# johnnyjana730/MVIN

Measured on AMD Instinct MI355X. Metric: (user,item) pairs scored/sec @ dim=64 hop=2 fan-out=32; % HBM roofline, higher is better.
Workload: dtype f32

## Files before the change

mvin_amd/csrc/mvin_fused_agg.hip:

```cpp
#include "mvin_fused_agg.h"

namespace mvin {

template <int K>
__global__ __launch_bounds__(kAggWaves * 64) void entity_aggregates_kernel(EntityAggArgs a) {
    constexpr int D = 64, SPL = K / 16;
    static_assert(K == 16 || K == 32 || K == 64, "K");
    extern __shared__ __attribute__((aligned(16))) float smem[];
    const int nRp = (a.nR + 3) & ~3;
    float* sT = smem;
    const int tid = threadIdx.x, lane = tid & 63, wave = tid >> 6;
    const int g = lane >> 4, c = lane & 15;
    unsigned* sLo = reinterpret_cast<unsigned*>(sT + nRp + wave * agg_list_words(K)) + g * (K + kAggPad);
    float* sLw = reinterpret_cast<float*>(reinterpret_cast<unsigned*>(sT + nRp + wave * agg_list_words(K)) + 4 * (K + kAggPad)) + g * (K + kAggPad);
    const bool att = a.t0 != nullptr;
    const float invK = 1.f / (float)K;
    const bool fast = agg_logit_table(a.t0, a.nR, sT, tid, lane);
    __syncthreads();

    const int tbytes = (int)a.table_bytes;
    const __amdgpu_buffer_rsrc_t tabS = __builtin_amdgcn_make_buffer_rsrc(const_cast<float*>(a.tabS), 0, tbytes, 0x00020000);
    const __amdgpu_buffer_rsrc_t tabG = __builtin_amdgcn_make_buffer_rsrc(const_cast<float*>(a.tabG), 0, tbytes, 0x00020000);
    const __amdgpu_buffer_rsrc_t selfS = __builtin_amdgcn_make_buffer_rsrc(const_cast<float*>(a.selfS), 0, a.selfS ? tbytes : 0, 0x00020000);
    const __amdgpu_buffer_rsrc_t selfG = __builtin_amdgcn_make_buffer_rsrc(const_cast<float*>(a.selfG), 0, tbytes, 0x00020000);
    const __amdgpu_buffer_rsrc_t adjE = __builtin_amdgcn_make_buffer_rsrc(const_cast<int32_t*>(a.adj_e), 0, (int)a.adj_bytes, 0x00020000);
    const __amdgpu_buffer_rsrc_t adjR = __builtin_amdgcn_make_buffer_rsrc(const_cast<int32_t*>(a.adj_r), 0, (int)a.adj_bytes, 0x00020000);
    const __amdgpu_buffer_rsrc_t outS = __builtin_amdgcn_make_buffer_rsrc(a.outS, 0, tbytes, 0x00020000);
    const __amdgpu_buffer_rsrc_t outG = __builtin_amdgcn_make_buffer_rsrc(a.outG, 0, tbytes, 0x00020000);
    const unsigned c16 = (unsigned)c * 16u;
    const unsigned n_entity = (unsigned)a.n_entity;
    const unsigned nquad = (n_entity + 3u) >> 2;

    auto run = [&](auto fast_tag) {
        constexpr bool FAST = decltype(fast_tag)::value;
        for (unsigned quad = blockIdx.x * kAggWaves + wave; quad < nquad; quad += gridDim.x * kAggWaves) {
            const unsigned e = quad * 4u + (unsigned)g;
            const bool valid = e < n_entity;
            unsigned ce[SPL], cr[SPL];
            agg_load_slots<SPL>(adjE, adjR, valid ? (e * (unsigned)K + (unsigned)(SPL * c)) * 4u : kAggOob, ce, cr);
            const unsigned so = valid ? e * (unsigned)(D * 4) + c16 : kAggPadRow;
            const float4 sg = agg_row4(selfG, so);
            const float4 ss = agg_row4(selfS, so);
            float wk[SPL];
            agg_row_weights<SPL, FAST>(cr, att, sT, (unsigned)(a.nR - 1), invK, wk);
            int cc = (int)(cr[0] >> 24);
            cc = valid ? (cc < 1 ? 1 : (cc > K ? K : cc)) : 0;
            __builtin_amdgcn_fence(__ATOMIC_RELEASE, "wavefront");
            __builtin_amdgcn_wave_barrier();
#pragma unroll
            for (int i = 0; i < SPL; ++i) {
                sLo[SPL * c + i] = ((cr[i] >> 16) & 0xFFu) ? (ce[i] & 0xFFFFFFu) * (unsigned)(D * 4) : kAggPadRow;
                sLw[SPL * c + i] = wk[i];
            }
            __builtin_amdgcn_fence(__ATOMIC_RELEASE, "wavefront");
            __builtin_amdgcn_wave_barrier();
            __builtin_amdgcn_fence(__ATOMIC_ACQUIRE, "wavefront");
            const int kmax = __builtin_amdgcn_readfirstlane(agg_xor32_imax(agg_xor16_imax(cc)));
            f32x2 s01 = {0.f, 0.f}, s23 = {0.f, 0.f}, g01 = {0.f, 0.f}, g23 = {0.f, 0.f};
            for (int k0 = 0; k0 < kmax; k0 += 4) {
                const uint4 o4 = *reinterpret_cast<const uint4*>(sLo + k0);
                const float4 w4 = *reinterpret_cast<const float4*>(sLw + k0);
                const unsigned off[4] = {o4.x, o4.y, o4.z, o4.w};
                const float ws_[4] = {w4.x, w4.y, w4.z, w4.w};
                float4 r1[4], r2[4];
#pragma unroll
                for (int t = 0; t < 4; ++t) {
                    r1[t] = agg_row4(tabS, off[t] + c16);
                    r2[t] = agg_row4(tabG, off[t] + c16);
                }
#pragma unroll
                for (int t = 0; t < 4; ++t) {
                    const f32x2 w2 = {ws_[t], ws_[t]};
                    s01 = __builtin_elementwise_fma(w2, f32x2{r1[t].x, r1[t].y}, s01);
                    s23 = __builtin_elementwise_fma(w2, f32x2{r1[t].z, r1[t].w}, s23);
                    g01 = __builtin_elementwise_fma(w2, f32x2{r2[t].x, r2[t].y}, g01);
                    g23 = __builtin_elementwise_fma(w2, f32x2{r2[t].z, r2[t].w}, g23);
                }
            }
            const unsigned oo = valid ? e * (unsigned)(D * 4) + c16 : kAggOob;
            const u32x4 vs = {__float_as_uint(s01[0] + ss.x), __float_as_uint(s01[1] + ss.y), __float_as_uint(s23[0] + ss.z),
                              __float_as_uint(s23[1] + ss.w)};
            const u32x4 vg = {__float_as_uint(g01[0] + sg.x), __float_as_uint(g01[1] + sg.y), __float_as_uint(g23[0] + sg.z),
                              __float_as_uint(g23[1] + sg.w)};
            __builtin_amdgcn_raw_buffer_store_b128(vs, outS, oo, 0, 0);
            __builtin_amdgcn_raw_buffer_store_b128(vg, outG, oo, 0, 0);
        }
    };
    if (fast) run(std::true_type{});
    else run(std::false_type{});
}

template <int K>
__global__ __launch_bounds__(kAggWaves * 64, K == 64 ? 3 : 4) void gather_attn_l2_agg_kernel(FusedL2Args a) {
    constexpr int D = 64, SPL = K / 16;
    static_assert(K == 16 || K == 32 || K == 64, "K");
    extern __shared__ __attribute__((aligned(16))) float smem[];
    const int nRp = (a.nR + 3) & ~3;
    float* sT = smem;
    const int tid = threadIdx.x, lane = tid & 63, wave = tid >> 6;
    const int g = lane >> 4, c = lane & 15;
    float* sUV = sT + nRp + wave * (16 * kAggUvLd + agg_list_words(K));
    unsigned* sLo = reinterpret_cast<unsigned*>(sUV + 16 * kAggUvLd) + g * (K + kAggPad);
    float* sLw = reinterpret_cast<float*>(reinterpret_cast<unsigned*>(sUV + 16 * kAggUvLd) + 4 * (K + kAggPad)) + g * (K + kAggPad);
    const bool att1 = a.t1 != nullptr;
    const float invK = 1.f / (float)K;
    const bool fold = a.fold != 0;
    const float c0 = fold ? 1.f : a.t0 != nullptr ? invK : 1.f;
    const bool fast = agg_logit_table(a.t1, a.nR, sT, tid, lane);
    __syncthreads();

    const unsigned tbytes = (unsigned)a.table_bytes;
    const __amdgpu_buffer_rsrc_t aggS = __builtin_amdgcn_make_buffer_rsrc(a.agg, 0, (int)tbytes, 0x00020000);
    const __amdgpu_buffer_rsrc_t aggG = __builtin_amdgcn_make_buffer_rsrc(reinterpret_cast<char*>(a.agg) + a.table_bytes, 0, (int)tbytes, 0x00020000);
    const __amdgpu_buffer_rsrc_t adjE = __builtin_amdgcn_make_buffer_rsrc(const_cast<int32_t*>(a.adj_e), 0, (int)a.adj_bytes, 0x00020000);
    const __amdgpu_buffer_rsrc_t adjR = __builtin_amdgcn_make_buffer_rsrc(const_cast<int32_t*>(a.adj_r), 0, (int)a.adj_bytes, 0x00020000);
    const __amdgpu_buffer_rsrc_t out0 = __builtin_amdgcn_make_buffer_rsrc(a.nagg0, 0, (int)(a.P * D * 4), 0x00020000);
    const __amdgpu_buffer_rsrc_t out1 = __builtin_amdgcn_make_buffer_rsrc(a.nagg1, 0, (int)(a.P * D * 4), 0x00020000);
    const unsigned c16 = (unsigned)c * 16u;
    if (c < kAggPad) {
        sLo[K + c] = kAggPadRow;
        sLw[K + c] = 0.f;
    }

    const int64_t nbatch = (a.P + 15) >> 4;
    const int64_t nwaves = (int64_t)gridDim.x * kAggWaves;
    auto run = [&](auto fast_tag) {
        constexpr bool FAST = decltype(fast_tag)::value;
        for (int64_t batch = (int64_t)blockIdx.x * kAggWaves + wave; batch < nbatch; batch += nwaves) {
            const int64_t p_base = batch << 4;
            int64_t pr = min(p_base + c, a.P - 1);
            if (a.order) pr = a.order[pr];
            const int x0c = fused_parent_id(a, pr);
            {
                const unsigned qoff = (unsigned)(pr / a.parents_per_pair) * (unsigned)(D * 4) + (unsigned)g * 16u;
                const char* qbase = reinterpret_cast<const char*>(a.q);
                float4 qb[4];
#pragma unroll
                for (int nt = 0; nt < 4; ++nt) qb[nt] = *reinterpret_cast<const float4*>(qbase + 64 * nt + (size_t)qoff);
                unsigned woff = ((unsigned)(4 * g) * (unsigned)D + (unsigned)c) * 4u;
                unsigned boff = (unsigned)g * 16u;
                asm volatile("" : "+v"(woff), "+v"(boff));
#pragma unroll
                for (int mat = 0; mat < 2; ++mat) {
                    const char* W = reinterpret_cast<const char*>(mat == 0 ? a.W1 : a.W2);
                    const char* bias = reinterpret_cast<const char*>(mat == 0 ? a.b1 : a.b2);
                    f32x4 acc[4];
#pragma unroll
                    for (int ntp = 0; ntp < 4; ++ntp) {
                        const float4 b = bias ? *reinterpret_cast<const float4*>(bias + 64 * ntp + (size_t)boff) : make_float4(0.f, 0.f, 0.f, 0.f);
                        acc[ntp] = f32x4{b.x, b.y, b.z, b.w};
                    }
#pragma unroll
                    for (int nt = 0; nt < 4; ++nt) {
                        const float bv[4] = {qb[nt].x, qb[nt].y, qb[nt].z, qb[nt].w};
#pragma unroll
                        for (int r = 0; r < 4; ++r) {
#pragma unroll
                            for (int ntp = 0; ntp < 4; ++ntp) {
                                const float w = *reinterpret_cast<const float*>(W + ((16 * nt + r) * D + 16 * ntp) * 4 + (size_t)woff);
                                acc[ntp] = __builtin_amdgcn_mfma_f32_16x16x4f32(w, bv[r], acc[ntp], 0, 0, 0);
                            }
                        }
                    }
#pragma unroll
                    for (int ntp = 0; ntp < 4; ++ntp)
                        *reinterpret_cast<float4*>(sUV + c * kAggUvLd + mat * D + 16 * ntp + 4 * g) = make_float4(acc[ntp][0], acc[ntp][1], acc[ntp][2], acc[ntp][3]);
                }
            }
            __builtin_amdgcn_fence(__ATOMIC_RELEASE, "wavefront");
            __builtin_amdgcn_wave_barrier();
            __builtin_amdgcn_fence(__ATOMIC_ACQUIRE, "wavefront");

            const int nquad = (int)((min((int64_t)16, a.P - p_base) + 3) >> 2);
            struct Quad {
                unsigned p;
                unsigned ce[SPL], cr[SPL];
                float4 s0;
            };
            auto quad_load = [&](int it) -> Quad {
                Quad qd;
                const int src = ((lane & 48) + 4 * it + g) << 2;
                qd.p = (unsigned)__builtin_amdgcn_ds_bpermute(src, (int)pr);
                const unsigned x0 = (unsigned)__builtin_amdgcn_ds_bpermute(src, x0c);
                agg_load_slots<SPL>(adjE, adjR, (x0 * (unsigned)K + (unsigned)(SPL * c)) * 4u, qd.ce, qd.cr);
                qd.s0 = agg_row4(aggS, x0 * (unsigned)(D * 4) + c16);
                return qd;
            };
            Quad nx = quad_load(0);
            for (int it = 0; it < nquad; ++it) {
                const int j = 4 * it + g;
                const bool pvalid = p_base + j < a.P;
                const Quad qd = nx;
                if (it + 1 < nquad) nx = quad_load(it + 1);
                const unsigned p = qd.p;
                const unsigned (&ce)[SPL] = qd.ce;
                const unsigned (&cr)[SPL] = qd.cr;
                const float4 s0 = qd.s0;
                const float4 u1 = *reinterpret_cast<const float4*>(sUV + j * kAggUvLd + 4 * c);
                const float4 vv = *reinterpret_cast<const float4*>(sUV + j * kAggUvLd + D + 4 * c);
                float wk[SPL];
                agg_row_weights<SPL, FAST>(cr, att1, sT, (unsigned)(a.nR - 1), invK, wk);
                int cc = (int)(cr[0] >> 24);
                cc = pvalid ? (cc < 1 ? 1 : (cc > K ? K : cc)) : 0;
                __builtin_amdgcn_fence(__ATOMIC_RELEASE, "wavefront");
                __builtin_amdgcn_wave_barrier();
#pragma unroll
                for (int i = 0; i < SPL; ++i) {
                    sLo[SPL * c + i] = ((cr[i] >> 16) & 0xFFu) ? (ce[i] & 0xFFFFFFu) * (unsigned)(D * 4) : kAggPadRow;
                    sLw[SPL * c + i] = wk[i];
                }
                __builtin_amdgcn_fence(__ATOMIC_RELEASE, "wavefront");
                __builtin_amdgcn_wave_barrier();
                __builtin_amdgcn_fence(__ATOMIC_ACQUIRE, "wavefront");
                const int kmax = __builtin_amdgcn_readfirstlane(agg_xor32_imax(agg_xor16_imax(cc)));
                const f32x2 v01 = {vv.x, vv.y}, v23 = {vv.z, vv.w};
                f32x2 a01 = {0.f, 0.f}, a23 = {0.f, 0.f};
                float4 ra[4], rb[4];
                float4 wa, wb;
                auto issue = [&](int k, float4 (&r)[4], float4& w) {
                    const uint4 o4 = *reinterpret_cast<const uint4*>(sLo + k);
                    w = *reinterpret_cast<const float4*>(sLw + k);
                    r[0] = agg_row4(aggG, o4.x + c16), r[1] = agg_row4(aggG, o4.y + c16);
                    r[2] = agg_row4(aggG, o4.z + c16), r[3] = agg_row4(aggG, o4.w + c16);
                };
                auto sum4 = [&](const float4 (&r)[4], const float4& w) {
                    const float ws_[4] = {w.x, w.y, w.z, w.w};
#pragma unroll
                    for (int t = 0; t < 4; ++t) {
                        const f32x2 o01 = f32x2{r[t].x, r[t].y} + v01, o23 = f32x2{r[t].z, r[t].w} + v23;
                        const f32x2 w2 = {ws_[t], ws_[t]};
                        a01 = __builtin_elementwise_fma(w2, f32x2{fmaxf(o01[0], 0.f), fmaxf(o01[1], 0.f)}, a01);
                        a23 = __builtin_elementwise_fma(w2, f32x2{fmaxf(o23[0], 0.f), fmaxf(o23[1], 0.f)}, a23);
                    }
                };
                issue(0, ra, wa);
                for (int k0 = 0; k0 < kmax; k0 += 8) {
                    issue(k0 + 4, rb, wb);
                    __builtin_amdgcn_sched_barrier(0);
                    sum4(ra, wa);
                    __builtin_amdgcn_sched_barrier(0);
                    issue(k0 + 8, ra, wa);
                    __builtin_amdgcn_sched_barrier(0);
                    sum4(rb, wb);
                    __builtin_amdgcn_sched_barrier(0);
                }
                const unsigned oo = pvalid ? p * (unsigned)(D * 4) + c16 : kAggOob;
                float4 r0 = make_float4(fmaf(c0, u1.x, s0.x), fmaf(c0, u1.y, s0.y), fmaf(c0, u1.z, s0.z), fmaf(c0, u1.w, s0.w));
                float4 r1 = make_float4(a01[0], a01[1], a23[0], a23[1]);
                if (fold) {
                    r0 = make_float4(fmaxf(r0.x, 0.f), fmaxf(r0.y, 0.f), fmaxf(r0.z, 0.f), fmaxf(r0.w, 0.f));
                    r1 = make_float4(r1.x + r0.x, r1.y + r0.y, r1.z + r0.z, r1.w + r0.w);
                }
                const u32x4 o0 = {__float_as_uint(r0.x), __float_as_uint(r0.y), __float_as_uint(r0.z), __float_as_uint(r0.w)};
                const u32x4 o1 = {__float_as_uint(r1.x), __float_as_uint(r1.y), __float_as_uint(r1.z), __float_as_uint(r1.w)};
                __builtin_amdgcn_raw_buffer_store_b128(o0, out0, oo, 0, 0);
                __builtin_amdgcn_raw_buffer_store_b128(o1, out1, oo, 0, 0);
            }
            __builtin_amdgcn_fence(__ATOMIC_RELEASE, "wavefront");
            __builtin_amdgcn_wave_barrier();
            __builtin_amdgcn_fence(__ATOMIC_ACQUIRE, "wavefront");
        }
    };
    if (fast) run(std::true_type{});
    else run(std::false_type{});
}

constexpr int kFoldTraceBatches = 16, kFoldTraceSlots = 20;
__device__ long long g_fold_trace[kFoldTraceBatches * kFoldTraceSlots];

template <int K, int MODE, bool TRACE = false>
__global__ __launch_bounds__(kAggWaves * 64, 3) void score_l2_folded_kernel(FoldArgs a) {
    constexpr int D = 64, SPL = K / 16;
    constexpr bool PIPE = MODE > 0, db = MODE == 2;
    constexpr int lb = db ? agg_list_words(K) : 0;
    static_assert(K == 16 || K == 32 || K == 64, "K");
    extern __shared__ __attribute__((aligned(16))) float smem[];
    const int nRp = (a.nR + 3) & ~3;
    float* sT = smem;
    const int tid = threadIdx.x, lane = tid & 63, wave = __builtin_amdgcn_readfirstlane(tid >> 6);
    const int g = lane >> 4, c = lane & 15;
    float* sUV = sT + nRp + wave * (16 * kAggUvLd + agg_list_words(K) + lb);
    unsigned* sLo = reinterpret_cast<unsigned*>(sUV + 16 * kAggUvLd) + g * (K + kAggPad);
    float* sLw = reinterpret_cast<float*>(reinterpret_cast<unsigned*>(sUV + 16 * kAggUvLd) + 4 * (K + kAggPad)) + g * (K + kAggPad);
    const bool att1 = a.t1 != nullptr;
    const float invK = 1.f / (float)K;
    const unsigned rmax = (unsigned)(a.nR - 1);
    const bool fast = agg_logit_table(a.t1, a.nR, sT, tid, lane);
    __syncthreads();

    const int tbytes = (int)a.table_bytes;
    const __amdgpu_buffer_rsrc_t aggS = __builtin_amdgcn_make_buffer_rsrc(const_cast<float*>(a.agg), 0, tbytes, 0x00020000);
    const __amdgpu_buffer_rsrc_t aggG = __builtin_amdgcn_make_buffer_rsrc(reinterpret_cast<char*>(const_cast<float*>(a.agg)) + a.table_bytes, 0, tbytes, 0x00020000);
    const __amdgpu_buffer_rsrc_t adjE = __builtin_amdgcn_make_buffer_rsrc(const_cast<int32_t*>(a.adj_e), 0, (int)a.adj_bytes, 0x00020000);
    const __amdgpu_buffer_rsrc_t adjR = __builtin_amdgcn_make_buffer_rsrc(const_cast<int32_t*>(a.adj_r), 0, (int)a.adj_bytes, 0x00020000);
    const unsigned c16 = (unsigned)c * 16u;
    if (c < kAggPad) {
        sLo[K + c] = kAggPadRow, sLo[lb + K + c] = kAggPadRow;
        sLw[K + c] = 0.f, sLw[lb + K + c] = 0.f;
    }

    const int64_t nbatch = (a.B + 15) >> 4;
    const int64_t nwaves = (int64_t)gridDim.x * kAggWaves;
    int traced = 0;
    auto stamp = [&](int slot, bool drain) {
        if constexpr (TRACE) {
            if (drain) asm volatile("s_waitcnt vmcnt(0)" ::: "memory");
            if (blockIdx.x == 0 && tid == 0 && traced < kFoldTraceBatches) g_fold_trace[traced * kFoldTraceSlots + slot] = __builtin_readcyclecounter();
        }
    };
    auto run = [&](auto fast_tag) {
        constexpr bool FAST = decltype(fast_tag)::value;
        const int lane = (int)__builtin_amdgcn_mbcnt_hi(~0u, __builtin_amdgcn_mbcnt_lo(~0u, 0u)), g = lane >> 4, c = lane & 15;
        unsigned* sLo = reinterpret_cast<unsigned*>(sUV + 16 * kAggUvLd) + g * (K + kAggPad);
        float* sLw = reinterpret_cast<float*>(reinterpret_cast<unsigned*>(sUV + 16 * kAggUvLd) + 4 * (K + kAggPad)) + g * (K + kAggPad);
        const unsigned c16 = (unsigned)c * 16u;
        unsigned xn = 0;
        f32x4 qn[4];
        auto fetch_batch = [&](int64_t b) {
            const int64_t prn = min((min(b, nbatch - 1) << 4) + c, a.B - 1);
            xn = (unsigned)a.items[prn * a.pid_stride];
            const char* qrow = reinterpret_cast<const char*>(a.q) + (size_t)((unsigned)prn * (unsigned)(D * 4) + (unsigned)g * 16u);
#pragma unroll
            for (int nt = 0; nt < 4; ++nt) qn[nt] = *reinterpret_cast<const f32x4*>(qrow + 64 * nt);
        };
        if constexpr (PIPE) fetch_batch((int64_t)blockIdx.x * kAggWaves + wave);
        for (int64_t batch = (int64_t)blockIdx.x * kAggWaves + wave; batch < nbatch; batch += nwaves) {
            const int64_t p_base = batch << 4;
            stamp(0, false);
            const int64_t pr = min(p_base + c, a.B - 1);
            const bool cvalid = p_base + c < a.B;
            unsigned x0u;
            if constexpr (PIPE) x0u = xn;
            else x0u = (unsigned)a.items[pr * a.pid_stride];
            x0u = x0u < a.max_id ? x0u : a.max_id;
            const int x0c = (int)x0u;
            unsigned woff = ((unsigned)(4 * g) * (unsigned)D + (unsigned)c * 4u) * 4u;
            unsigned boff = (unsigned)g * 16u;
            unsigned roff = (unsigned)pr * (unsigned)(D * 4) + (unsigned)g * 16u;
            asm volatile("" : "+v"(woff), "+v"(boff));
            auto chain = [&](auto np_, auto&& wsel, auto&& bsel, auto&& asel, auto&& between, auto&& late) {
                constexpr int NP = decltype(np_)::value, T = 4 * NP;
                __amdgpu_buffer_rsrc_t wr[NP];
                static_for<NP>([&](auto j_) {
                    const float* Wp = wsel(j_);
                    asm volatile("" : "+s"(Wp));
                    wr[decltype(j_)::value] = __builtin_amdgcn_make_buffer_rsrc(const_cast<float*>(Wp), 0, D * D * 4, 0x00020000);
                });
                f32x4 ring[3][4];
                auto load = [&](auto s_) {
                    constexpr int s = decltype(s_)::value, j = s / 4, nt = s % 4;
#pragma unroll
                    for (int r = 0; r < 4; ++r) {
                        const u32x4 v = __builtin_amdgcn_raw_buffer_load_b128(wr[j], woff + (unsigned)(r * D * 4), nt * 16 * D * 4, 0);
                        ring[s % 3][r] = f32x4{__uint_as_float(v[0]), __uint_as_float(v[1]), __uint_as_float(v[2]), __uint_as_float(v[3])};
                    }
                };
                load(std::integral_constant<int, 0>{});
                load(std::integral_constant<int, 1>{});
                static_for<T>([&](auto s_) {
                    constexpr int s = decltype(s_)::value, j = s / 4, nt = s % 4;
                    if constexpr (s + 2 < T) load(std::integral_constant<int, s + 2>{});
                    if constexpr (s >= T - 3) late(std::integral_constant<int, s - (T - 3)>{});
                    __builtin_amdgcn_sched_barrier(0);
                    const f32x4 (&b)[4] = bsel(std::integral_constant<int, j>{});
                    f32x4 (&acc)[4] = asel(std::integral_constant<int, j>{});
#pragma unroll
                    for (int r = 0; r < 4; ++r) {
#pragma unroll
                        for (int ntp = 0; ntp < 4; ++ntp) acc[ntp] = __builtin_amdgcn_mfma_f32_16x16x4f32(ring[s % 3][r][ntp], b[nt][r], acc[ntp], 0, 0, 0);
                    }
                    __builtin_amdgcn_sched_barrier(0);
                    if constexpr (nt == 3) between(std::integral_constant<int, j>{});
                });
            };
            auto bias4 = [&](const float* bp, f32x4 (&acc)[4]) {
                const char* bias = reinterpret_cast<const char*>(bp);
#pragma unroll
                for (int ntp = 0; ntp < 4; ++ntp)
                    acc[ntp] = bias ? *reinterpret_cast<const f32x4*>(bias + 64 * ntp + (size_t)boff) : f32x4{0.f, 0.f, 0.f, 0.f};
            };
            struct Quad {
                unsigned ce[SPL], cr[SPL];
                float4 s0;
            };
            auto quad_load = [&](int it) -> Quad {
                Quad qd;
                const unsigned x0 = (unsigned)__builtin_amdgcn_ds_bpermute(((lane & 48) + 4 * it + g) << 2, x0c);
                agg_load_slots<SPL>(adjE, adjR, (x0 * (unsigned)K + (unsigned)(SPL * c)) * 4u, qd.ce, qd.cr);
                qd.s0 = agg_row4(aggS, x0 * (unsigned)(D * 4) + c16);
                return qd;
            };
            Quad q0, q1;
            auto late1 = [&](auto s_) {
                if constexpr (PIPE && decltype(s_)::value == 0) q0 = quad_load(0), q1 = quad_load(1);
            };
            f32x4 qm[4], qb[4];
            {
                const char* qbase = reinterpret_cast<const char*>(a.q);
#pragma unroll
                for (int nt = 0; nt < 4; ++nt) {
                    if constexpr (PIPE) qb[nt] = qn[nt];
                    else qb[nt] = *reinterpret_cast<const f32x4*>(qbase + 64 * nt + (size_t)roff);
                }
                stamp(1, true);
                f32x4 at[4], av[4];
                bias4(a.bq, at);
                bias4(a.bv, av);
                auto store_tv = [&](auto j_) {
                    constexpr int j = decltype(j_)::value;
                    if constexpr (j < 2) {
                        const f32x4 (&acc)[4] = j == 0 ? at : av;
#pragma unroll
                        for (int ntp = 0; ntp < 4; ++ntp) *reinterpret_cast<f32x4*>(sUV + c * kAggUvLd + j * D + 16 * ntp + 4 * g) = acc[ntp];
                    }
                };
                bias4(a.bm, qm);
                if (a.dbg & 4) late1(std::integral_constant<int, 0>{});
                else
                    chain(std::integral_constant<int, 3>{}, [&](auto j_) { return decltype(j_)::value == 0 ? a.Wq : decltype(j_)::value == 1 ? a.Wv : a.Wqm; },
                          [&](auto) -> const f32x4 (&)[4] { return qb; },
                          [&](auto j_) -> f32x4 (&)[4] {
                              if constexpr (decltype(j_)::value == 0) return at;
                              else if constexpr (decltype(j_)::value == 1) return av;
                              else return qm;
                          }, store_tv, late1);
            }
            __builtin_amdgcn_fence(__ATOMIC_RELEASE, "wavefront");
            __builtin_amdgcn_wave_barrier();
            __builtin_amdgcn_fence(__ATOMIC_ACQUIRE, "wavefront");
            stamp(2, false);

            const int nquad = (a.dbg & 8) ? 0 : (int)((min((int64_t)16, a.B - p_base) + 3) >> 2);
            auto issue = [&](const unsigned* lo, int k, float4 (&r)[4]) {
                const uint4 o4 = *reinterpret_cast<const uint4*>(lo + k);
                r[0] = agg_row4(aggG, o4.x + c16), r[1] = agg_row4(aggG, o4.y + c16);
                r[2] = agg_row4(aggG, o4.z + c16), r[3] = agg_row4(aggG, o4.w + c16);
            };
            auto sum4 = [&](const float4 (&r)[4], const float4& w, const f32x2 v01, const f32x2 v23, f32x2& a01, f32x2& a23) {
                const float ws_[4] = {w.x, w.y, w.z, w.w};
#pragma unroll
                for (int t = 0; t < 4; ++t) {
                    const f32x2 o01 = f32x2{r[t].x, r[t].y} + v01, o23 = f32x2{r[t].z, r[t].w} + v23;
                    const f32x2 w2 = {ws_[t], ws_[t]};
                    a01 = __builtin_elementwise_fma(w2, f32x2{fmaxf(o01[0], 0.f), fmaxf(o01[1], 0.f)}, a01);
                    a23 = __builtin_elementwise_fma(w2, f32x2{fmaxf(o23[0], 0.f), fmaxf(o23[1], 0.f)}, a23);
                }
            };
            auto lists = [&](const Quad& qd, int it, int ob) -> int {
                const bool pvalid = p_base + 4 * it + g < a.B;
                float wk[SPL];
                agg_row_weights<SPL, FAST>(qd.cr, att1, sT, rmax, invK, wk);
                int cc = (int)(qd.cr[0] >> 24);
                cc = pvalid ? (cc < 1 ? 1 : (cc > K ? K : cc)) : 0;
                __builtin_amdgcn_fence(__ATOMIC_RELEASE, "wavefront");
                __builtin_amdgcn_wave_barrier();
#pragma unroll
                for (int i = 0; i < SPL; ++i) {
                    sLo[ob + SPL * c + i] = ((qd.cr[i] >> 16) & 0xFFu) ? (qd.ce[i] & 0xFFFFFFu) * (unsigned)(D * 4) : kAggPadRow;
                    sLw[ob + SPL * c + i] = wk[i];
                }
                __builtin_amdgcn_fence(__ATOMIC_RELEASE, "wavefront");
                __builtin_amdgcn_wave_barrier();
                __builtin_amdgcn_fence(__ATOMIC_ACQUIRE, "wavefront");
                return (a.dbg & 1) ? 0 : __builtin_amdgcn_readfirstlane(agg_xor32_imax(agg_xor16_imax(cc)));
            };
            if constexpr (PIPE) {
                int kmax = lists(q0, 0, 0);
                for (int it = 0; it < nquad; ++it) {
                    stamp(3 + 3 * it, false);
                    const int cur = (it & 1) ? lb : 0;
                    float* rowT = sUV + (4 * it + g) * kAggUvLd + 4 * c;
                    const float4 vv = *reinterpret_cast<const float4*>(rowT + D);
                    const f32x2 v01 = {vv.x, vv.y}, v23 = {vv.z, vv.w};
                    f32x2 a01 = {0.f, 0.f}, a23 = {0.f, 0.f};
                    const int kr = (kmax + 7) & ~7;
                    float4 r0[4], r1[4], r2[4];
                    auto wts = [&](int k) { return *reinterpret_cast<const float4*>(sLw + cur + k); };
                    const float4 s0 = q0.s0;
                    if (it > 0 && it + 1 < nquad) q1 = quad_load(it + 1);
                    issue(sLo + cur, 0, r0);
                    issue(sLo + cur, 4, r1);
                    if (kr > 8) issue(sLo + cur, 8, r2);
                    stamp(4 + 3 * it, true);
                    __builtin_amdgcn_sched_barrier(0);
                    int kmax_n = 0;
                    if (db && it + 1 < nquad) kmax_n = lists(q1, it + 1, lb - cur);
                    __builtin_amdgcn_sched_barrier(0);
                    for (int k0 = 0; k0 < kr; k0 += 24) {
                        sum4(r0, wts(k0), v01, v23, a01, a23);
                        __builtin_amdgcn_sched_barrier(0);
                        if (k0 + 12 < kr) issue(sLo + cur, k0 + 12, r0);
                        __builtin_amdgcn_sched_barrier(0);
                        sum4(r1, wts(k0 + 4), v01, v23, a01, a23);
                        __builtin_amdgcn_sched_barrier(0);
                        if (k0 + 8 < kr) {
                            if (k0 + 16 < kr) issue(sLo + cur, k0 + 16, r1);
                            __builtin_amdgcn_sched_barrier(0);
                            sum4(r2, wts(k0 + 8), v01, v23, a01, a23);
                            __builtin_amdgcn_sched_barrier(0);
                            if (k0 + 16 < kr) issue(sLo + cur, k0 + 20, r2);
                            __builtin_amdgcn_sched_barrier(0);
                            sum4(r0, wts(k0 + 12), v01, v23, a01, a23);
                            __builtin_amdgcn_sched_barrier(0);
                            if (k0 + 16 < kr) {
                                if (k0 + 24 < kr) issue(sLo + cur, k0 + 24, r0);
                                __builtin_amdgcn_sched_barrier(0);
                                sum4(r1, wts(k0 + 16), v01, v23, a01, a23);
                                __builtin_amdgcn_sched_barrier(0);
                                if (k0 + 24 < kr) issue(sLo + cur, k0 + 28, r1);
                                __builtin_amdgcn_sched_barrier(0);
                                sum4(r2, wts(k0 + 20), v01, v23, a01, a23);
                                __builtin_amdgcn_sched_barrier(0);
                                if (k0 + 32 < kr) issue(sLo + cur, k0 + 32, r2);
                                __builtin_amdgcn_sched_barrier(0);
                            }
                        }
                    }
                    const float4 tt = *reinterpret_cast<const float4*>(rowT);
                    const float4 o0 = make_float4(fmaxf(s0.x + tt.x, 0.f), fmaxf(s0.y + tt.y, 0.f), fmaxf(s0.z + tt.z, 0.f), fmaxf(s0.w + tt.w, 0.f));
                    *reinterpret_cast<float4*>(rowT) = o0;
                    *reinterpret_cast<float4*>(rowT + D) = make_float4(a01[0] + o0.x, a01[1] + o0.y, a23[0] + o0.z, a23[1] + o0.w);
                    if (!db && it + 1 < nquad) kmax_n = lists(q1, it + 1, 0);
                    kmax = kmax_n;
                    q0 = q1;
                    stamp(5 + 3 * it, false);
                }
            } else {
                Quad nx = quad_load(0);
                for (int it = 0; it < nquad; ++it) {
                    stamp(3 + 3 * it, false);
                    const Quad qd = nx;
                    if (it + 1 < nquad) nx = quad_load(it + 1);
                    float* rowT = sUV + (4 * it + g) * kAggUvLd + 4 * c;
                    const float4 tt = *reinterpret_cast<const float4*>(rowT);
                    const float4 vv = *reinterpret_cast<const float4*>(rowT + D);
                    const int kmax = lists(qd, it, 0);
                    const f32x2 v01 = {vv.x, vv.y}, v23 = {vv.z, vv.w};
                    f32x2 a01 = {0.f, 0.f}, a23 = {0.f, 0.f};
                    float4 ra[4], rb[4];
                    float4 wa, wb;
                    auto wts = [&](int k) { return *reinterpret_cast<const float4*>(sLw + k); };
                    issue(sLo, 0, ra), wa = wts(0);
                    if constexpr (TRACE) {
                        issue(sLo, 4, rb), wb = wts(4);
                        stamp(4 + 3 * it, true);
                    }
                    for (int k0 = 0; k0 < kmax; k0 += 8) {
                        if (!TRACE || k0 > 0) issue(sLo, k0 + 4, rb), wb = wts(k0 + 4);
                        __builtin_amdgcn_sched_barrier(0);
                        sum4(ra, wa, v01, v23, a01, a23);
                        __builtin_amdgcn_sched_barrier(0);
                        issue(sLo, k0 + 8, ra), wa = wts(k0 + 8);
                        __builtin_amdgcn_sched_barrier(0);
                        sum4(rb, wb, v01, v23, a01, a23);
                        __builtin_amdgcn_sched_barrier(0);
                    }
                    const float4 o0 = make_float4(fmaxf(qd.s0.x + tt.x, 0.f), fmaxf(qd.s0.y + tt.y, 0.f), fmaxf(qd.s0.z + tt.z, 0.f),
                                                  fmaxf(qd.s0.w + tt.w, 0.f));
                    *reinterpret_cast<float4*>(rowT) = o0;
                    *reinterpret_cast<float4*>(rowT + D) = make_float4(a01[0] + o0.x, a01[1] + o0.y, a23[0] + o0.z, a23[1] + o0.w);
                    stamp(5 + 3 * it, false);
                }
            }
            __builtin_amdgcn_fence(__ATOMIC_RELEASE, "wavefront");
            __builtin_amdgcn_wave_barrier();
            __builtin_amdgcn_fence(__ATOMIC_ACQUIRE, "wavefront");
            {
                f32x4 zb[4], ob[4], o2[4], m0r[4], uor[4];
                auto m0_load = [&]() {
#pragma unroll
                    for (int ntp = 0; ntp < 4; ++ntp)
                        m0r[ntp] = *reinterpret_cast<const f32x4*>(reinterpret_cast<const char*>(a.M0) + (size_t)x0u * (D * 4) + 64 * ntp + (size_t)boff);
                };
                auto uo_load = [&]() {
#pragma unroll
                    for (int ntp = 0; ntp < 4; ++ntp)
                        uor[ntp] = *reinterpret_cast<const f32x4*>(reinterpret_cast<const char*>(a.user_o) + 64 * ntp + (size_t)roff);
                };
                auto late2 = [&](auto s_) {
                    if constexpr (PIPE && decltype(s_)::value == 0) m0_load();
                    if constexpr (PIPE && decltype(s_)::value == 1) fetch_batch(batch + nwaves);
                    if constexpr (PIPE && decltype(s_)::value == 2) uo_load();
                };
#pragma unroll
                for (int nt = 0; nt < 4; ++nt) zb[nt] = *reinterpret_cast<const f32x4*>(sUV + c * kAggUvLd + D + 16 * nt + 4 * g);
                bias4(a.a1, o2);
                auto relu_o2 = [&]() {
#pragma unroll
                    for (int nt = 0; nt < 4; ++nt) o2[nt] = f32x4{fmaxf(o2[nt][0], 0.f), fmaxf(o2[nt][1], 0.f), fmaxf(o2[nt][2], 0.f), fmaxf(o2[nt][3], 0.f)};
                };
                auto read_ob = [&]() {
#pragma unroll
                    for (int nt = 0; nt < 4; ++nt) ob[nt] = *reinterpret_cast<const f32x4*>(sUV + c * kAggUvLd + 16 * nt + 4 * g);
                };
                if (a.dbg & 2) late2(std::integral_constant<int, 0>{}), late2(std::integral_constant<int, 1>{}), late2(std::integral_constant<int, 2>{});
                else
                    chain(std::integral_constant<int, 3>{}, [&](auto j_) { constexpr int j = decltype(j_)::value; return j == 0 ? a.A1 : j == 1 ? a.Wm1 : a.Wm2; },
                          [&](auto j_) -> const f32x4 (&)[4] {
                              constexpr int j = decltype(j_)::value;
                              if constexpr (j == 0) return zb;
                              else if constexpr (j == 1) return ob;
                              else return o2;
                          },
                          [&](auto j_) -> f32x4 (&)[4] { if constexpr (decltype(j_)::value == 0) return o2; else return qm; },
                          [&](auto j_) {
                              if constexpr (decltype(j_)::value == 0) relu_o2(), read_ob();
                          }, late2);
                stamp(15, false);
                if constexpr (!PIPE) m0_load();
                stamp(16, true);
                if constexpr (!PIPE) {
                    if (a.user_o != a.q) uo_load();
                    else
#pragma unroll
                        for (int ntp = 0; ntp < 4; ++ntp) uor[ntp] = qb[ntp];
                }
                float part = 0.f;
#pragma unroll
                for (int ntp = 0; ntp < 4; ++ntp) {
                    const f32x4 uo = uor[ntp];
                    const f32x4 it4 = qm[ntp] + m0r[ntp];
                    if (a.item_emb && cvalid) *reinterpret_cast<f32x4*>(reinterpret_cast<char*>(a.item_emb) + 64 * ntp + (size_t)roff) = it4;
                    part += it4[0] * uo[0] + it4[1] * uo[1] + it4[2] * uo[2] + it4[3] * uo[3];
                }
                part = xor32_sum(xor16_sum(part));
                if (g == 0 && cvalid) {
                    a.scores[pr] = part;
                    if (a.sig) a.sig[pr] = 1.f / (1.f + expf(-part));
                }
                stamp(17, false);
            }
            __builtin_amdgcn_fence(__ATOMIC_RELEASE, "wavefront");
            __builtin_amdgcn_wave_barrier();
            __builtin_amdgcn_fence(__ATOMIC_ACQUIRE, "wavefront");
            if constexpr (TRACE) ++traced;
        }
    };
    if (fast) run(std::true_type{});
    else run(std::false_type{});
}

hipError_t fold_read_trace(long long* host_dst, size_t n) {
    const size_t have = sizeof(g_fold_trace) / sizeof(long long);
    return hipMemcpyFromSymbol(host_dst, HIP_SYMBOL(g_fold_trace), (n < have ? n : have) * sizeof(long long));
}

template <int K>
static hipError_t launch_fold_k(const FoldArgs& a, hipStream_t st) {
    static const bool pipe = !(getenv("MVIN_FOLD_PIPE") && atoi(getenv("MVIN_FOLD_PIPE")) == 0);
    static const bool trace = getenv("MVIN_FOLD_TRACE") != nullptr;
    static const int grid_cap = getenv("MVIN_FOLD_GRID") ? atoi(getenv("MVIN_FOLD_GRID")) : 0;
    static const int wgs = getenv("MVIN_FOLD_WGS") ? atoi(getenv("MVIN_FOLD_WGS")) : 0;
    using Kern = void (*)(FoldArgs);
    constexpr size_t kLdsNoOptIn = 48 * 1024;
    constexpr bool kTwoLists = fused_agg_lds_words(0, K) * sizeof(float) + (size_t)kAggWaves * agg_list_words(K) * sizeof(float) <= kLdsNoOptIn;
    auto kernel_of = [&](int mode) -> Kern {
        if (trace) {
            if constexpr (kTwoLists) {
                if (mode == 2) return score_l2_folded_kernel<K, 2, true>;
            }
            return mode ? (Kern)score_l2_folded_kernel<K, 1, true> : (Kern)score_l2_folded_kernel<K, 0, true>;
        }
        if constexpr (kTwoLists) {
            if (mode == 2) return score_l2_folded_kernel<K, 2, false>;
        }
        return mode ? (Kern)score_l2_folded_kernel<K, 1, false> : (Kern)score_l2_folded_kernel<K, 0, false>;
    };
    struct Plan {
        int dev, nR, per_cu;
        size_t lds;
        Kern kern;
    };
    static thread_local Plan plan{-1, -1, 0, 0, nullptr};
    int dev = 0;
    if (hipGetDevice(&dev) != hipSuccess) return hipGetLastError();
    if (plan.dev != dev || plan.nR != a.nR) {
        auto occupancy = [&](Kern k, size_t lds) {
            const int v = workgroups_per_cu(k, kAggWaves * 64, lds, 0);
            return v > 8 ? 8 : v;
        };
        const size_t lds1 = fused_agg_lds_bytes(a.nR, K), lds2 = lds1 + (size_t)kAggWaves * agg_list_words(K) * sizeof(float);
        const int mode1 = pipe ? 1 : 0;
        const int occ1 = occupancy(kernel_of(mode1), lds1);
        const int occ2 = pipe && kTwoLists && lds2 <= kLdsNoOptIn ? occupancy(kernel_of(2), lds2) : 0;
        const bool two = occ2 > 0 && occ2 >= occ1;
        plan.kern = kernel_of(two ? 2 : mode1);
        plan.lds = two ? lds2 : lds1;
        plan.per_cu = two ? occ2 : occ1 > 0 ? occ1 : 4;
        if (wgs > 0) plan.per_cu = wgs;
        plan.dev = dev, plan.nR = a.nR;
        if (getenv("MVIN_FOLD_REPORT"))
            fprintf(stderr, "score_l2_folded_kernel<%d>: mode %d, LDS %zu bytes per workgroup, %d workgroups per CU\n", K, two ? 2 : mode1, plan.lds, plan.per_cu);
    }
    const int64_t nbatch = (a.B + 15) >> 4;
    const int64_t want = (nbatch + kAggWaves - 1) / kAggWaves;
    int64_t grid = persistent_grid(want, plan.per_cu);
    if (grid_cap > 0 && grid_cap < grid) grid = grid_cap;
    plan.kern<<<(int)grid, kAggWaves * 64, plan.lds, st>>>(a);
    return hipGetLastError();
}

hipError_t launch_score_l2_folded(const float* agg, const float* M0, const int32_t* adj_e, const int32_t* adj_r, const int32_t* items, int pid_stride,
                                  const float* t1, const float* q, const float* user_o, const float* Wq, const float* bq, const float* Wv,
                                  const float* bv, const float* Wqm, const float* A1, const float* a1, const float* Wm1, const float* Wm2,
                                  const float* bm, float* item_emb, float* scores, float* sig, int64_t B, int K, int D, int nR, int n_entity,
                                  hipStream_t st) {
    FoldArgs f{};
    f.agg = agg, f.M0 = M0, f.adj_e = adj_e, f.adj_r = adj_r, f.items = items, f.pid_stride = pid_stride, f.t1 = t1, f.q = q, f.user_o = user_o;
    f.Wq = Wq, f.bq = bq, f.Wv = Wv, f.bv = bv, f.Wqm = Wqm, f.A1 = A1, f.a1 = a1, f.Wm1 = Wm1, f.Wm2 = Wm2, f.bm = bm;
    f.item_emb = item_emb, f.scores = scores, f.sig = sig, f.B = B, f.K = K, f.nR = nR, f.max_id = (unsigned)(n_entity - 1);
    f.table_bytes = (uint64_t)n_entity * (uint64_t)D * 4, f.adj_bytes = (uint64_t)n_entity * (uint64_t)K * 4;
    static const char* dbg = getenv("MVIN_FOLD_DBG");
    f.dbg = dbg ? atoi(dbg) : 0;
    if (D == 32) return launch_score_l2_folded_d32(f, st);
    switch (K) {
        case 16: return launch_fold_k<16>(f, st);
        case 32: return launch_fold_k<32>(f, st);
        case 64: return launch_fold_k<64>(f, st);
        default: return hipErrorInvalidValue;
    }
}

bool fused_agg_supported(int D, int K) { return D == 64 && (K == 16 || K == 32 || K == 64); }
bool fused_fold_supported(int D, int K) { return fused_agg_supported(D, K) || (D == 32 && (K == 16 || K == 32)); }
size_t fused_fold_d32_lds_bytes(int nR, int K);
size_t fused_fold_lds_bytes(int D, int nR, int K) { return D == 32 ? fused_fold_d32_lds_bytes(nR, K) : fused_agg_lds_bytes(nR, K); }

size_t fused_agg_lds_bytes(int nR, int K) { return fused_agg_lds_words(nR, K) * sizeof(float); }

bool fused_agg_applies(const FusedL2Args& a, int D) {
    return a.prj && fused_agg_supported(D, a.K) && !a.probs_parent && !a.probs_child && a.adj_r && a.adj_bytes > 0 &&
           a.adj_bytes < (1ull << 31) && a.table_bytes > 0 && a.table_bytes < (1ull << 30) && (uint64_t)a.P * D * 4 < (1ull << 31) &&
           a.max_id < (1u << 24) && a.nR > 0 && fused_agg_lds_bytes(a.nR, a.K) <= 48 * 1024;
}

template <int K>
static hipError_t launch_entity_aggregates_k(const EntityAggArgs& a, hipStream_t st) {
    const size_t lds = ((size_t)((a.nR + 3) & ~3) + (size_t)kAggWaves * agg_list_words(K)) * sizeof(float);
    const int64_t nquad = ((int64_t)a.n_entity + 3) >> 2;
    const int64_t want = (nquad + kAggWaves - 1) / kAggWaves;
    entity_aggregates_kernel<K><<<(int)persistent_grid(want, 8), kAggWaves * 64, lds, st>>>(a);
    return hipGetLastError();
}

hipError_t launch_entity_aggregates(const EntityAggArgs& a, hipStream_t st) {
    if (a.D == 32) return launch_entity_aggregates_d32(a, st);
    switch (a.K) {
        case 16: return launch_entity_aggregates_k<16>(a, st);
        case 32: return launch_entity_aggregates_k<32>(a, st);
        case 64: return launch_entity_aggregates_k<64>(a, st);
        default: return hipErrorInvalidValue;
    }
}

__global__ void fold_prepare_kernel(const float* __restrict__ W0, const float* __restrict__ b0, const float* __restrict__ W1,
                                    const float* __restrict__ b1, const float* __restrict__ W2, const float* __restrict__ b2,
                                    const float* __restrict__ A0, const float* __restrict__ a0, const float* __restrict__ Wmix,
                                    const float* __restrict__ bmix, const float* __restrict__ A1, float c, int D, float* __restrict__ blk) {
    const int i = blockIdx.x, j = threadIdx.x;
    float* Wstack = blk;
    float* Wv = blk + (size_t)4 * D * D;
    float* Wq = Wv + (size_t)D * D;
    float* bv = Wq + (size_t)D * D;
    float* bq = bv + D;
    float* bm = bq + D;
    if (j >= D) return;
    float s0 = 0.f, s1 = 0.f, s2 = 0.f, sm = 0.f;
    for (int k0 = 0; k0 < D; k0 += 8) {
        float av[8], mv[8], x0[8], x1[8], x2[8];
#pragma unroll
        for (int k = 0; k < 8; ++k) {
            av[k] = A0[(size_t)(k0 + k) * D + j];
            mv[k] = Wmix[(size_t)(k0 + k) * D + j];
            x0[k] = i < D ? W0[(size_t)i * D + k0 + k] : (b0 ? b0[k0 + k] : 0.f);
            x1[k] = i < D ? W1[(size_t)i * D + k0 + k] : (b1 ? b1[k0 + k] : 0.f);
            x2[k] = i < D ? W2[(size_t)i * D + k0 + k] : (b2 ? b2[k0 + k] : 0.f);
        }
#pragma unroll
        for (int k = 0; k < 8; ++k) {
            s0 = fmaf(x0[k], av[k], s0);
            s1 = fmaf(x1[k], av[k], s1);
            s2 = fmaf(x2[k], av[k], s2);
            sm = fmaf(x0[k], mv[k], sm);
        }
    }
    if (i < D) {
        Wstack[(size_t)i * D + j] = s1;
        Wstack[(size_t)D * D + (size_t)i * D + j] = s2;
        Wstack[(size_t)2 * D * D + (size_t)i * D + j] = s0;
        Wstack[(size_t)3 * D * D + (size_t)i * D + j] = sm;
        Wv[(size_t)i * D + j] = fmaf(c, s2, s1);
        Wq[(size_t)i * D + j] = fmaf(c, s1, s0);
        if (D == 64 || D == 32) {
            float* Wperm = bm + D;
            const size_t o = (size_t)i * D + (size_t)(j & 15) * (D / 16) + (size_t)(j >> 4);
            const size_t DD = (size_t)D * D;
            Wperm[o] = fmaf(c, s1, s0);
            Wperm[DD + o] = fmaf(c, s2, s1);
            Wperm[2 * DD + o] = sm;
            Wperm[3 * DD + o] = A1[(size_t)i * D + j];
            Wperm[4 * DD + o] = Wmix[DD + (size_t)i * D + j];
            Wperm[5 * DD + o] = Wmix[2 * DD + (size_t)i * D + j];
        }
    } else {
        const float av0 = a0 ? a0[j] : 0.f;
        bv[j] = fmaf(c, s2, s1) + av0;
        bq[j] = fmaf(c, s1, s0) + av0;
        bm[j] = (bmix ? bmix[j] : 0.f) + sm;
    }
}

hipError_t launch_fold_prepare(const float* W0, const float* b0, const float* W1, const float* b1, const float* W2, const float* b2, const float* A0,
                               const float* a0, const float* Wmix, const float* bmix, const float* A1, float c, int D, float* blk, hipStream_t st) {
    fold_prepare_kernel<<<D + 1, D < 64 ? 64 : D, 0, st>>>(W0, b0, W1, b1, W2, b2, A0, a0, Wmix, bmix, A1, c, D, blk);
    return hipGetLastError();
}

template <int K>
static hipError_t launch_agg_k(const FusedL2Args& a, hipStream_t st) {
    const size_t lds = fused_agg_lds_bytes(a.nR, K);
    const int v = workgroups_per_cu(gather_attn_l2_agg_kernel<K>, kAggWaves * 64, lds, 4);
    const int64_t nbatch = (a.P + 15) >> 4;
    const int64_t want = (nbatch + kAggWaves - 1) / kAggWaves;
    gather_attn_l2_agg_kernel<K><<<(int)persistent_grid(want, v > 8 ? 8 : v), kAggWaves * 64, lds, st>>>(a);
    return hipGetLastError();
}

hipError_t launch_gather_attn_l2_agg(const FusedL2Args& a, hipStream_t st) {
    switch (a.K) {
        case 16: return launch_agg_k<16>(a, st);
        case 32: return launch_agg_k<32>(a, st);
        case 64: return launch_agg_k<64>(a, st);
        default: return hipErrorInvalidValue;
    }
}

}
```

Baseline: 545.5 million.

## Sort wave pairs by neighbor-list length and trim gather loop granularity

Each 16-pair batch now reads each item's adjacency length word and ranks the pairs by length within the group using readlane comparisons. It then permutes item ids with ds_permute so every quad of four pairs holds similar-length lists, and the per-quad loop bound (the max length across the quad) wastes fewer masked gather iterations. Invalid tail pairs are sorted to the front and skipped by starting the quad loop at it0. The gather loop step drops from 8/24 to 4/12 elements with guarded sum4 calls to cut padding. The cost is an extra dependent buffer load, 16 readlanes and permutes per batch, indirect sUV row addressing, and more branches in the inner loop.

```diff
diff --git a/mvin_amd/csrc/mvin_fused_agg.hip b/mvin_amd/csrc/mvin_fused_agg.hip
--- a/mvin_amd/csrc/mvin_fused_agg.hip
+++ b/mvin_amd/csrc/mvin_fused_agg.hip
@@ -334,6 +334,9 @@
             else x0u = (unsigned)a.items[pr * a.pid_stride];
             x0u = x0u < a.max_id ? x0u : a.max_id;
             const int x0c = (int)x0u;
+            const unsigned len_word = __builtin_amdgcn_raw_buffer_load_b32(adjR, x0u * (unsigned)(K * 4), 0, 0);
+            const int ninv = 16 - (int)min((int64_t)16, a.B - p_base);
+            const int it0 = (a.dbg & 8) ? 4 : ninv >> 2;
             unsigned woff = ((unsigned)(4 * g) * (unsigned)D + (unsigned)c * 4u) * 4u;
             unsigned boff = (unsigned)g * 16u;
             unsigned roff = (unsigned)pr * (unsigned)(D * 4) + (unsigned)g * 16u;
@@ -383,16 +386,30 @@
                 unsigned ce[SPL], cr[SPL];
                 float4 s0;
             };
+            int xs = 0, pm = 0;
+            auto deal = [&]() {
+                int len = (int)(len_word >> 24);
+                len = len < 1 ? 1 : (len > K ? K : len);
+                const int key = cvalid ? (len << 4 | c) : c;
+                int rank = 0;
+#pragma unroll
+                for (int i = 0; i < 16; ++i) rank += __builtin_amdgcn_readlane(key, i) < key ? 1 : 0;
+                const int dst = ((lane & 48) + rank) << 2;
+                xs = __builtin_amdgcn_ds_permute(dst, x0c);
+                pm = __builtin_amdgcn_ds_permute(dst, c);
+            };
             auto quad_load = [&](int it) -> Quad {
                 Quad qd;
-                const unsigned x0 = (unsigned)__builtin_amdgcn_ds_bpermute(((lane & 48) + 4 * it + g) << 2, x0c);
+                const unsigned x0 = (unsigned)__builtin_amdgcn_ds_bpermute(((lane & 48) + 4 * it + g) << 2, xs);
                 agg_load_slots<SPL>(adjE, adjR, (x0 * (unsigned)K + (unsigned)(SPL * c)) * 4u, qd.ce, qd.cr);
                 qd.s0 = agg_row4(aggS, x0 * (unsigned)(D * 4) + c16);
                 return qd;
             };
+            auto pair_of = [&](int it) { return __builtin_amdgcn_ds_bpermute(((lane & 48) + 4 * it + g) << 2, pm); };
             Quad q0, q1;
             auto late1 = [&](auto s_) {
-                if constexpr (PIPE && decltype(s_)::value == 0) q0 = quad_load(0), q1 = quad_load(1);
+                if constexpr (PIPE && decltype(s_)::value == 0) deal();
+                if constexpr (PIPE && decltype(s_)::value == 1) q0 = quad_load(it0 & 3), q1 = quad_load(min(it0 + 1, 3));
             };
             f32x4 qm[4], qb[4];
             {
@@ -415,7 +432,7 @@
                     }
                 };
                 bias4(a.bm, qm);
-                if (a.dbg & 4) late1(std::integral_constant<int, 0>{});
+                if (a.dbg & 4) late1(std::integral_constant<int, 0>{}), late1(std::integral_constant<int, 1>{});
                 else
                     chain(std::integral_constant<int, 3>{}, [&](auto j_) { return decltype(j_)::value == 0 ? a.Wq : decltype(j_)::value == 1 ? a.Wv : a.Wqm; },
                           [&](auto) -> const f32x4 (&)[4] { return qb; },
@@ -430,7 +447,6 @@
             __builtin_amdgcn_fence(__ATOMIC_ACQUIRE, "wavefront");
             stamp(2, false);
 
-            const int nquad = (a.dbg & 8) ? 0 : (int)((min((int64_t)16, a.B - p_base) + 3) >> 2);
             auto issue = [&](const unsigned* lo, int k, float4 (&r)[4]) {
                 const uint4 o4 = *reinterpret_cast<const uint4*>(lo + k);
                 r[0] = agg_row4(aggG, o4.x + c16), r[1] = agg_row4(aggG, o4.y + c16);
@@ -446,8 +462,12 @@
                     a23 = __builtin_elementwise_fma(w2, f32x2{fmaxf(o23[0], 0.f), fmaxf(o23[1], 0.f)}, a23);
                 }
             };
+            auto zero4 = [&](float4 (&r)[4]) {
+#pragma unroll
+                for (int t = 0; t < 4; ++t) r[t] = make_float4(0.f, 0.f, 0.f, 0.f);
+            };
             auto lists = [&](const Quad& qd, int it, int ob) -> int {
-                const bool pvalid = p_base + 4 * it + g < a.B;
+                const bool pvalid = 4 * it + g >= ninv;
                 float wk[SPL];
                 agg_row_weights<SPL, FAST>(qd.cr, att1, sT, rmax, invK, wk);
                 int cc = (int)(qd.cr[0] >> 24);
@@ -465,53 +485,42 @@
                 return (a.dbg & 1) ? 0 : __builtin_amdgcn_readfirstlane(agg_xor32_imax(agg_xor16_imax(cc)));
             };
             if constexpr (PIPE) {
-                int kmax = lists(q0, 0, 0);
-                for (int it = 0; it < nquad; ++it) {
+                int kmax = it0 < 4 ? lists(q0, it0, (it0 & 1) ? lb : 0) : 0;
+                for (int it = it0; it < 4; ++it) {
                     stamp(3 + 3 * it, false);
                     const int cur = (it & 1) ? lb : 0;
-                    float* rowT = sUV + (4 * it + g) * kAggUvLd + 4 * c;
+                    float* rowT = sUV + pair_of(it) * kAggUvLd + 4 * c;
                     const float4 vv = *reinterpret_cast<const float4*>(rowT + D);
                     const f32x2 v01 = {vv.x, vv.y}, v23 = {vv.z, vv.w};
                     f32x2 a01 = {0.f, 0.f}, a23 = {0.f, 0.f};
-                    const int kr = (kmax + 7) & ~7;
+                    const int kr = (kmax + 3) & ~3;
                     float4 r0[4], r1[4], r2[4];
                     auto wts = [&](int k) { return *reinterpret_cast<const float4*>(sLw + cur + k); };
                     const float4 s0 = q0.s0;
-                    if (it > 0 && it + 1 < nquad) q1 = quad_load(it + 1);
+                    if (it > it0 && it + 1 < 4) q1 = quad_load(it + 1);
                     issue(sLo + cur, 0, r0);
-                    issue(sLo + cur, 4, r1);
-                    if (kr > 8) issue(sLo + cur, 8, r2);
+                    if (4 < kr) issue(sLo + cur, 4, r1);
+                    else zero4(r1);
+                    if (8 < kr) issue(sLo + cur, 8, r2);
                     stamp(4 + 3 * it, true);
                     __builtin_amdgcn_sched_barrier(0);
                     int kmax_n = 0;
-                    if (db && it + 1 < nquad) kmax_n = lists(q1, it + 1, lb - cur);
+                    if (db && it + 1 < 4) kmax_n = lists(q1, it + 1, lb - cur);
                     __builtin_amdgcn_sched_barrier(0);
-                    for (int k0 = 0; k0 < kr; k0 += 24) {
+                    for (int k0 = 0; k0 < kr; k0 += 12) {
                         sum4(r0, wts(k0), v01, v23, a01, a23);
                         __builtin_amdgcn_sched_barrier(0);
                         if (k0 + 12 < kr) issue(sLo + cur, k0 + 12, r0);
                         __builtin_amdgcn_sched_barrier(0);
-                        sum4(r1, wts(k0 + 4), v01, v23, a01, a23);
-                        __builtin_amdgcn_sched_barrier(0);
-                        if (k0 + 8 < kr) {
+                        if (k0 + 4 < kr) {
+                            sum4(r1, wts(k0 + 4), v01, v23, a01, a23);
+                            __builtin_amdgcn_sched_barrier(0);
                             if (k0 + 16 < kr) issue(sLo + cur, k0 + 16, r1);
                             __builtin_amdgcn_sched_barrier(0);
-                            sum4(r2, wts(k0 + 8), v01, v23, a01, a23);
-                            __builtin_amdgcn_sched_barrier(0);
-                            if (k0 + 16 < kr) issue(sLo + cur, k0 + 20, r2);
-                            __builtin_amdgcn_sched_barrier(0);
-                            sum4(r0, wts(k0 + 12), v01, v23, a01, a23);
-                            __builtin_amdgcn_sched_barrier(0);
-                            if (k0 + 16 < kr) {
-                                if (k0 + 24 < kr) issue(sLo + cur, k0 + 24, r0);
+                            if (k0 + 8 < kr) {
+                                sum4(r2, wts(k0 + 8), v01, v23, a01, a23);
                                 __builtin_amdgcn_sched_barrier(0);
-                                sum4(r1, wts(k0 + 16), v01, v23, a01, a23);
-                                __builtin_amdgcn_sched_barrier(0);
-                                if (k0 + 24 < kr) issue(sLo + cur, k0 + 28, r1);
-                                __builtin_amdgcn_sched_barrier(0);
-                                sum4(r2, wts(k0 + 20), v01, v23, a01, a23);
-                                __builtin_amdgcn_sched_barrier(0);
-                                if (k0 + 32 < kr) issue(sLo + cur, k0 + 32, r2);
+                                if (k0 + 20 < kr) issue(sLo + cur, k0 + 20, r2);
                                 __builtin_amdgcn_sched_barrier(0);
                             }
                         }
@@ -520,21 +529,22 @@
                     const float4 o0 = make_float4(fmaxf(s0.x + tt.x, 0.f), fmaxf(s0.y + tt.y, 0.f), fmaxf(s0.z + tt.z, 0.f), fmaxf(s0.w + tt.w, 0.f));
                     *reinterpret_cast<float4*>(rowT) = o0;
                     *reinterpret_cast<float4*>(rowT + D) = make_float4(a01[0] + o0.x, a01[1] + o0.y, a23[0] + o0.z, a23[1] + o0.w);
-                    if (!db && it + 1 < nquad) kmax_n = lists(q1, it + 1, 0);
+                    if (!db && it + 1 < 4) kmax_n = lists(q1, it + 1, 0);
                     kmax = kmax_n;
                     q0 = q1;
                     stamp(5 + 3 * it, false);
                 }
             } else {
-                Quad nx = quad_load(0);
-                for (int it = 0; it < nquad; ++it) {
+                deal();
+                Quad nx = quad_load(it0 & 3);
+                for (int it = it0; it < 4; ++it) {
                     stamp(3 + 3 * it, false);
                     const Quad qd = nx;
-                    if (it + 1 < nquad) nx = quad_load(it + 1);
-                    float* rowT = sUV + (4 * it + g) * kAggUvLd + 4 * c;
+                    if (it + 1 < 4) nx = quad_load(it + 1);
+                    float* rowT = sUV + pair_of(it) * kAggUvLd + 4 * c;
                     const float4 tt = *reinterpret_cast<const float4*>(rowT);
                     const float4 vv = *reinterpret_cast<const float4*>(rowT + D);
-                    const int kmax = lists(qd, it, 0);
+                    const int kr = (lists(qd, it, 0) + 3) & ~3;
                     const f32x2 v01 = {vv.x, vv.y}, v23 = {vv.z, vv.w};
                     f32x2 a01 = {0.f, 0.f}, a23 = {0.f, 0.f};
                     float4 ra[4], rb[4];
@@ -542,18 +552,23 @@
                     auto wts = [&](int k) { return *reinterpret_cast<const float4*>(sLw + k); };
                     issue(sLo, 0, ra), wa = wts(0);
                     if constexpr (TRACE) {
-                        issue(sLo, 4, rb), wb = wts(4);
+                        if (4 < kr) issue(sLo, 4, rb), wb = wts(4);
+                        else zero4(rb);
                         stamp(4 + 3 * it, true);
                     }
-                    for (int k0 = 0; k0 < kmax; k0 += 8) {
-                        if (!TRACE || k0 > 0) issue(sLo, k0 + 4, rb), wb = wts(k0 + 4);
+                    for (int k0 = 0; k0 < kr; k0 += 8) {
+                        const bool second = k0 + 4 < kr;
+                        if ((!TRACE || k0 > 0) && second) issue(sLo, k0 + 4, rb), wb = wts(k0 + 4);
+                        else if (!TRACE) zero4(rb);
                         __builtin_amdgcn_sched_barrier(0);
                         sum4(ra, wa, v01, v23, a01, a23);
                         __builtin_amdgcn_sched_barrier(0);
-                        issue(sLo, k0 + 8, ra), wa = wts(k0 + 8);
-                        __builtin_amdgcn_sched_barrier(0);
-                        sum4(rb, wb, v01, v23, a01, a23);
-                        __builtin_amdgcn_sched_barrier(0);
+                        if (second) {
+                            if (k0 + 8 < kr) issue(sLo, k0 + 8, ra), wa = wts(k0 + 8);
+                            __builtin_amdgcn_sched_barrier(0);
+                            sum4(rb, wb, v01, v23, a01, a23);
+                            __builtin_amdgcn_sched_barrier(0);
+                        }
                     }
                     const float4 o0 = make_float4(fmaxf(qd.s0.x + tt.x, 0.f), fmaxf(qd.s0.y + tt.y, 0.f), fmaxf(qd.s0.z + tt.z, 0.f),
                                                   fmaxf(qd.s0.w + tt.w, 0.f));
```

Measured after the change: 553.6 million (median of 6 runs). 1.01x the previous value.
